# simplerr/rust-renderer

Measured on AMD Instinct MI355X. Metric: Mrays/s (path rays: primary + bounce + sun-shadow + light-shadow) at 1920x1080, 20 spp = 20 frames x 1 spp; camera and sun at rest, the one-off builds of the camera grid and the sun grid outside the timed region (value_with_grid_builds charges them to these frames, value_tree_walk uses neither grid), higher is better.
Workload: dtype f32

## Files before the change

### rust-renderer_amd/csrc/context.hip

```cpp
#include <hip/hip_runtime.h>
#include <rccl/rccl.h>
#include <dlfcn.h>

#include <algorithm>
#include <atomic>
#include <chrono>
#include <cstdlib>
#include <cmath>
#include <cstdio>
#include <cstring>
#include <string>
#include <thread>
#include <vector>

#include "bvh.h"
#include "context_internal.h"
#include "context_state.h"
#include "device_scan.h"
#include "device_types.h"
#include "utopian_hip.h"

using namespace uh;

namespace {
std::string g_create_error;
}

int fail(uh_ctx* c, int code, const std::string& msg) {
   if (c)
      c->err = msg;
   else
      g_create_error = msg;
   return code;
}

namespace {

void begin_timed(uh_ctx* c, int kind, hipStream_t stream = nullptr) {
   if (!stream) stream = c->stream;
   if (!c->time_kernels) return;
   EventPair ep;
   if (!c->free_events.empty()) {
      ep = c->free_events.back();
      c->free_events.pop_back();
   } else {
      (void)hipEventCreate(&ep.start);
      (void)hipEventCreate(&ep.stop);
   }
   ep.kind = kind;
   (void)hipEventRecord(ep.start, stream);
   c->pending.push_back(ep);
}
void end_timed(uh_ctx* c, hipStream_t stream = nullptr) {
   if (!c->time_kernels) return;
   (void)hipEventRecord(c->pending.back().stop, stream ? stream : c->stream);
}
void drain_timed(uh_ctx* c) {
   for (EventPair& ep : c->pending) {
      float ms = 0.0f;
      if (hipEventSynchronize(ep.stop) == hipSuccess && hipEventElapsedTime(&ms, ep.start, ep.stop) == hipSuccess) {
         c->ms_by_kind[ep.kind] += ms;
         if (ep.kind == 0) c->trace_closest_launches++;
         if (ep.kind == 4) c->trace_light_launches++;
      }
      c->free_events.push_back(ep);
   }
   c->pending.clear();
}

}

LaunchCfg cfg(uh_ctx* c) {
// ... 132 lines not shown
   c->d_meshes.release();
   c->d_obj_corners.release();
   c->d_world_corners.release();
   c->d_node_box.release();
   c->d_refit_meshes.release();
   c->d_src.release();
   c->d_tex.release();
   c->d_lut.release();
   c->d_sun_cells.release();
   c->d_sun_entries.release();
   c->d_sun_recs.release();
   c->d_sun_coarse.release();
   c->d_cam_cells.release();
   c->d_cam_entries.release();
   c->accumulation.release();
   c->gbuffer.release();
   c->output.release();
   for (auto& r : c->reservoirs) r.release();
   c->dstats.release();
   for (HostMesh& m : c->meshes) {
      if (m.d_verts) (void)hipFree(m.d_verts);
      if (m.d_indices) (void)hipFree(m.d_indices);
   }
   for (hipEvent_t ev : c->mupd.ev)
      if (ev) (void)hipEventDestroy(ev);
   c->mupd.table.release();
   c->mupd.flag.release();
   for (hipEvent_t ev : {c->iso.begin, c->iso.end})
      if (ev) (void)hipEventDestroy(ev);
   c->iso.counts.release();
   c->iso.chunks.release();
   c->iso.box.release();
   c->iso.total.release();
   destroy_graphs(c);
   for (auto& s : c->slots) s.destroy();
   for (hipEvent_t ev : c->ev_band)
      if (ev) (void)hipEventDestroy(ev);
   if (c->restir_stream) {
      for (hipEvent_t ev : {c->ev_restir, c->rs_start, c->rs_stop})
         if (ev) (void)hipEventDestroy(ev);
      (void)hipStreamDestroy(c->restir_stream);
      c->restir_stream = nullptr;
   }
   c->owned_pixels.release();
   c->tile_send.release();
   c->tile_recv.release();
   if (c->ev_compose) (void)hipEventDestroy(c->ev_compose);
   delete c;
}

int uh_add_texture_rgba8(uh_ctx* c, const uint8_t* pixels, uint32_t w, uint32_t h, uint32_t* out_index) {
   if (!c) return UH_ERR_INVALID_ARGUMENT;
   if (!pixels || !w || !h) return fail(c, UH_ERR_INVALID_ARGUMENT, "uh_add_texture_rgba8: null or empty texture");
   HIP_TRY(c, hipSetDevice(c->device));
   uchar4* dev = nullptr;
   HIP_TRY(c, hipMalloc((void**)&dev, (size_t)w * h * 4));
   const uint32_t tiles_x = (w % 8 == 0 && h % 8 == 0) ? w / 8 : 0;
   std::vector<uint8_t> tiled;
   const uint8_t* src = pixels;
   if (tiles_x) {
      tiled.resize((size_t)w * h * 4);
      for (uint32_t y = 0; y < h; y++)
         for (uint32_t x = 0; x < w; x++) {
            size_t at = ((size_t)((y >> 3) * tiles_x + (x >> 3)) << 6) + ((y & 7) << 3) + (x & 7);
            std::memcpy(&tiled[at * 4], &pixels[((size_t)y * w + x) * 4], 4);
         }
      src = tiled.data();
   }
   hipError_t e = hipMemcpy(dev, src, (size_t)w * h * 4, hipMemcpyHostToDevice);
   if (e != hipSuccess) {
      (void)hipFree(dev);
      return fail(c, UH_ERR_HIP, std::string("texture upload: ") + hipGetErrorString(e));
   }
   c->textures.push_back(uh_ctx::HostTex{w, h, dev, tiles_x});
   c->built = false;
   if (out_index) *out_index = (uint32_t)c->textures.size() - 1;
   return UH_OK;
}

int uh_add_light(uh_ctx* c, const UhGpuLight* light, uint32_t* out_index) {
   if (!c) return UH_ERR_INVALID_ARGUMENT;
   if (!light) return fail(c, UH_ERR_INVALID_ARGUMENT, "uh_add_light: null light");
   if (c->lights.size() >= UH_MAX_GPU_LIGHTS) return fail(c, UH_ERR_CAPACITY, "uh_add_light: more than 1024 lights (MAX_NUM_GPU_LIGHTS)");
   c->lights.push_back(*light);
   c->built = false;
   c->topology_valid = false;
   if (out_index) *out_index = (uint32_t)c->lights.size() - 1;
   return UH_OK;
}

int uh_get_num_lights(uh_ctx* c, uint32_t* out) {
   if (!c || !out) return UH_ERR_INVALID_ARGUMENT;
   *out = (uint32_t)c->lights.size();
   return UH_OK;
}

extern "C++" FrameParams make_params(uh_ctx* c, const UhViewUniformData& v) {
   FrameParams fp;
   std::memset(&fp, 0, sizeof(fp));
   std::memcpy(fp.inv_view, v.inverse_view, sizeof(fp.inv_view));
   std::memcpy(fp.inv_proj, v.inverse_projection, sizeof(fp.inv_proj));
   std::memcpy(fp.prev_pv, v.prev_frame_projection_view, sizeof(fp.prev_pv));
   float d = (v.sun_dir[0] * v.sun_dir[0] + v.sun_dir[1] * v.sun_dir[1]) + v.sun_dir[2] * v.sun_dir[2];
   float inv = 1.0f / std::sqrt(d);
   for (int a = 0; a < 3; a++) fp.sun_dir[a] = v.sun_dir[a] * inv;
   fp.W = c->W;
   fp.H = c->H;
   fp.frame_number = (uint32_t)(int32_t)((float)v.total_samples + v.time * 10000.0f);
   fp.batch_frames = 1;
   fp.frame_numbers[0] = fp.frame_number;
   fp.total_samples_of[0] = v.total_samples;
   fp.samples_per_frame = v.samples_per_frame;
   fp.total_samples = v.total_samples;
   fp.num_bounces = v.num_bounces;
   fp.accumulation_limit = v.accumulation_limit;
   fp.sky_enabled = v.sky_enabled;
   fp.sun_shadow_enabled = v.sun_shadow_enabled;
   fp.lights_enabled = v.lights_enabled;
   fp.use_ris = v.use_ris_light_sampling;
   fp.full_frame_restir = c->full_frame_restir ? 1u : 0u;
   fp.furnace = c->furnace ? 1u : 0u;
   fp.num_lights_used = v.num_lights < v.max_num_lights_used ? v.num_lights : v.max_num_lights_used;
   fp.temporal_enabled = v.temporal_reuse_enabled;
   fp.spatial_enabled = v.spatial_reuse_enabled;
   fp.tp_rank = c->tp_rank;
   fp.tp_world = c->tp_world;
   fp.tp_tile = c->tp_tile;
// ... 856 lines not shown
   else if (n == "sun_grid_build") {
      c->sun_device_build = value != 0;
      c->sun_attempted = false;
   } else if (n == "sun_grid_density") {
      if (!range(1, 4096)) return bad("(entries per triangle) must be 1..4096");
      c->sun_limits.entries_per_triangle = (double)value;
      c->sun_attempted = false;
   } else if (n == "sun_grid_max_walk") {
      if (!range(1, 4096)) return bad("(longest list a ray tests itself) must be 1..4096");
      c->sun_limits.max_walk = (uint32_t)value;
      c->sun_attempted = false;
   } else if (n == "sun_grid_max_mb") {
      if (!range(1, 65536)) return bad("must be 1..65536");
      c->sun_limits.max_entries = ((uint64_t)value << 20) / sizeof(SunGridEntry);
      c->sun_attempted = false;
   } else if (n == "sun_grid_force") {
      const SunGridLimits defaults;
      c->sun_limits.max_mean_list = value ? 1e30 : defaults.max_mean_list;
      c->sun_limits.max_fallback_area = value ? 2.0 : defaults.max_fallback_area;
      c->sun_attempted = false;
   } else if (n == "sun_grid_inline_max_mb") {
      if (!range(-1, 1 << 20)) return bad("must be -1 (auto: 4 x the packet array), 0 (off) .. 1048576");
      c->sun_inline_max_mb = value;
      c->sun_attempted = false;
   } else if (n == "sun_verdicts")
      c->sun_verdicts = value != 0;
   else if (n == "sun_grid_coarse") {
      if (!range(0, 6)) return bad("(log2 of the block edge in cells) must be 0..6");
      c->sun_coarse_shift = (uint32_t)value;
      c->sun_attempted = false;
   }
   else if (n == "camera_grid")
      c->cam_grid_enabled = value != 0;
   else if (n == "camera_grid_max_walk") {
      if (!range(1, 4096)) return bad("must be 1..4096");
      c->cam_limits.max_walk = (uint32_t)value;
      c->cam_attempted = false;
   } else if (n == "camera_grid_walk_whole") {
      if (!range(0, 65536)) return bad("must be 0..65536");
      c->cam_walk_whole = (uint32_t)value;
      c->cam_attempted = false;
   } else if (n == "camera_grid_max_mean_list_x10") {
      if (!range(1, 100000)) return bad("must be 1..100000");
      c->cam_limits.max_mean_list = value / 10.0;
      c->cam_attempted = false;
   } else if (n == "primary_implicit")
      c->primary_implicit = value != 0;
   else if (n == "full_frame_restir")
      c->full_frame_restir = value != 0;
   else if (n == "iso_reference_triangulation")
      c->iso_reference = value != 0;
   else if (n == "furnace")
      c->furnace = value != 0;
   else if (n == "shadow_map_size") {
      if (!range(16, 8192)) return bad("must be 16..8192");
      if ((uint32_t)value != c->shadow_map_size) {
         if (int st = sync_all(c)) return st;
         c->hy.shadow_maps([](auto& b, size_t) { b.release(); });
         c->hy.s_bins.geom = 0;
         c->hy.smap_size = 0;
      }
      c->shadow_map_size = (uint32_t)value;
   }
   else if (n == "overlap")
      c->overlap_miss = c->overlap_shadow = value != 0;
   else if (n == "batch_frames") {
      if (!range(0, (int)kMaxBatchFrames)) return bad("must be 0 (auto) .. 32");
      c->batch_frames = (uint32_t)value;
   } else if (n == "frames_in_flight") {
      if (!range(1, (int)kMaxSlots)) return bad("must be 1..8");
      (void)sync_all(c);
      c->frames_in_flight = (uint32_t)value;
      c->next_slot = 0;
   } else if (n == "fused_bounces") {
      if (!range(-1, 8)) return bad("must be 0 (off), 1 (on when no frame is in flight), -1 (always on) or 2..8 (as 1, and blocks per CU of its grid)");
      c->fused_bounces = value != 0;
      c->fused_always = value == -1;
      if (value >= 2) c->fused_blocks_per_cu = (uint32_t)value;
   } else if (n == "trace_blocks_per_cu") {
      if (!range(1, 8)) return bad("must be 1..8");
      c->closest_blocks_per_cu = c->shadow_blocks_per_cu = (uint32_t)value;
   } else
      return fail(c, UH_ERR_INVALID_ARGUMENT, "unknown option: " + n);
   return UH_OK;
}

int uh_set_tile_partition(uh_ctx* c, uint32_t rank, uint32_t world, uint32_t tile_size) {
   if (!c) return UH_ERR_INVALID_ARGUMENT;
   if (world == 0 || rank >= world || tile_size == 0) return fail(c, UH_ERR_INVALID_ARGUMENT, "uh_set_tile_partition: need rank < world, tile_size > 0");
   HIP_TRY(c, hipSetDevice(c->device));
   if (int st = sync_all(c)) return st;
   c->tp_rank = rank;
   c->tp_world = world;
   c->tp_tile = tile_size;
   c->n_owned = c->W * c->H;
   c->owned_pixels.release();
   if (world > 1) {
      const uint32_t tiles_x = (c->W + tile_size - 1) / tile_size;
      std::vector<uint32_t> own;
      own.reserve((size_t)c->W * c->H / world + 1);
      for (uint32_t y = 0; y < c->H; y++)
         for (uint32_t x = 0; x < c->W; x++)
            if (((y / tile_size) * tiles_x + x / tile_size) % world == rank) own.push_back(y * c->W + x);
      c->n_owned = (uint32_t)own.size();
      HIP_TRY(c, c->owned_pixels.alloc(own.size() ? own.size() : 1));
      if (!own.empty()) HIP_TRY(c, hipMemcpy(c->owned_pixels.p, own.data(), own.size() * 4, hipMemcpyHostToDevice));
// ... 381 lines not shown
```

### rust-renderer_amd/csrc/context_state.h

```cpp
#pragma once
#include <hip/hip_runtime.h>

#include <string>
#include <utility>
#include <vector>

#include "bvh.h"
#include "context_internal.h"
#include "device_types.h"
#include "utopian_hip.h"

using namespace uh;

struct HostMesh {
   std::vector<UhVertex> vertices;
   std::vector<uint32_t> indices;
   UhGpuMaterial material;
   float o2w[12];
   float w2o[9];
   bool iso = false, iso_reference = true;
   uint32_t iso_res = 0;
   float iso_lo = 0.0f, iso_hi = 0.0f;
   bool dev = false, host_valid = true;
   UhVertex* d_verts = nullptr;
// ... 153 lines not shown
      radf.release();
      pixcol.release();
      for (auto& q : queues) q.release();
      sun_lit.release();
      control.release();
      for (hipEvent_t* ev : {&ev_traced, &ev_missed, &ev_shaded, &ev_shadowed, &ev_side_done, &ev_acc, &frame_start, &frame_stop}) {
         if (*ev) (void)hipEventDestroy(*ev);
         *ev = nullptr;
      }
      if (side) (void)hipStreamDestroy(side);
      if (stream) (void)hipStreamDestroy(stream);
      stream = side = nullptr;
      ready = false;
   }
};

constexpr uint32_t kRestirBatch = 16;
constexpr int kSpatialRing = 2 * (int)kRestirBatch + 1;

struct uh_ctx {
   int device = 0;
   Slot slots[kMaxSlots];
   uint32_t frames_in_flight = 4;
   uint32_t batch_frames = 0;
   uint32_t next_slot = 0;
   uint32_t shard_cap = 0;
   hipEvent_t last_acc = nullptr;
   hipStream_t restir_stream = nullptr;
   hipEvent_t ev_restir = nullptr, rs_start = nullptr, rs_stop = nullptr;
   bool restir_recorded = false;
   int spatial_cur = 0;
   hipEvent_t spatial_reader[kSpatialRing] = {};
   uint32_t rp_rank = 0, rp_world = 1, rp_band_rows = 0;
   size_t res_stride = 0;
   UhRestirExchangeFn rp_exchange = nullptr;
   void* rp_user = nullptr;
   hipEvent_t ev_band[kSpatialRing] = {};
   void* rccl = nullptr;
   hipEvent_t t_start = nullptr, t_stop = nullptr;
   Slot* last_slot = nullptr;
   hipStream_t& stream = slots[0].stream;
   PathState& ps = slots[0].ps;
   DevBuf<Control>& control = slots[0].control;
   bool overlap_miss = true, overlap_shadow = true;
   uint32_t W = 0, H = 0;
   uint32_t num_cus = 256;
   uint32_t closest_blocks_per_cu = 5, shadow_blocks_per_cu = 5;
   uint32_t cam_walk_whole = 512;
   bool fused_bounces = true;
   bool fused_always = false;
   static constexpr uint32_t kFusedMaxPaths = 4u << 20;
   uint32_t fused_blocks_per_cu = 4;
   static constexpr uint32_t kSingleFrameBlocksPerCu = 4;
   std::string err;

   std::vector<HostMesh> meshes;
   std::vector<UhGpuLight> lights;
   struct HostTex {
      uint32_t w, h;
      uchar4* dev;
      uint32_t tiles_x;
   };
   std::vector<HostTex> textures;
   bool built = false;

   DevBuf<float4> d_nodes, d_tris, d_shade, d_lights;
   DevBuf<MeshShade> d_meshes;
   DevBuf<float> d_obj_corners, d_world_corners, d_node_box;
   DevBuf<RefitMesh> d_refit_meshes;
   std::vector<uint32_t> packet_keys;
   std::vector<uint32_t> level_start;
   bool topology_valid = false;
   bool device_build = false, src_valid = false;
   uint32_t device_build_kind = 1;
   uint32_t ploc_sah_top = 1024;
   static constexpr uint32_t kPlocRadius = 8;
   BuildSources d_src;
   std::vector<uint32_t> src_tris;
   std::vector<uint64_t> src_serial;
   struct IsoUpdate {
      DevBuf<uint32_t> counts, chunks, box;
      DevBuf<unsigned long long> total;
      hipEvent_t begin = nullptr, end = nullptr;
      UhIsosurfaceUpdateStats st{};
   } iso;
   std::vector<uint64_t> packet_serial;
   struct MeshUpdate {
      DevBuf<DeformMesh> table;
      DevBuf<uint32_t> flag;
      hipEvent_t ev[3] = {nullptr, nullptr, nullptr};
      UhMeshUpdateStats st{};
   } mupd;
   float refit_ms = 0.0f;
   DevBuf<TexInfo> d_tex;
   DevBuf<float> d_lut;
   SceneDev scene{};

   DevBuf<float4> accumulation, gbuffer;
   DevBuf<uchar4> output;
   DevBuf<UhReservoir> reservoirs[3], spatial_ring;
   DevBuf<float4> gb_ray_o, gb_ray_d, gb_hit;
   DevBuf<DeviceStats> dstats;
   Images im{};

   bool count_visits = false, time_kernels = false, full_frame_restir = false;
   bool iso_reference = true;
   uint32_t shadow_map_size = 4096;
   bool furnace = false;
   uint64_t frames = 0;
   float build_ms = 0.0f, last_frame_ms = 0.0f;
   float ms_by_kind[5] = {0, 0, 0, 0, 0};
   uint32_t trace_closest_launches = 0, trace_light_launches = 0;
   bool frame_timed = false;
   std::vector<EventPair> pending, free_events;
// ... 159 lines not shown
```

### rust-renderer_amd/csrc/device_math.h

```cpp
#pragma once
#include <hip/hip_runtime.h>

#include "device_types.h"

namespace uh {

struct V3 {
   float x, y, z;
};
__device__ __forceinline__ V3 v3(float x, float y, float z) { return V3{x, y, z}; }
__device__ __forceinline__ V3 operator+(V3 a, V3 b) { return v3(a.x + b.x, a.y + b.y, a.z + b.z); }
__device__ __forceinline__ V3 operator-(V3 a, V3 b) { return v3(a.x - b.x, a.y - b.y, a.z - b.z); }
__device__ __forceinline__ V3 operator*(V3 a, V3 b) { return v3(a.x * b.x, a.y * b.y, a.z * b.z); }
__device__ __forceinline__ V3 operator*(V3 a, float s) { return v3(a.x * s, a.y * s, a.z * s); }
__device__ __forceinline__ V3 operator*(float s, V3 a) { return v3(s * a.x, s * a.y, s * a.z); }
__device__ __forceinline__ V3 vneg(V3 a) { return v3(-a.x, -a.y, -a.z); }
__device__ __forceinline__ float dot3(V3 a, V3 b) { return (a.x * b.x + a.y * b.y) + a.z * b.z; }
__device__ __forceinline__ float length3(V3 a) { return sqrtf(dot3(a, a)); }
__device__ __forceinline__ V3 normalize3(V3 a) {
   float inv = 1.0f / sqrtf(dot3(a, a));
   return a * inv;
}
__device__ __forceinline__ V3 xyz(float4 v) { return v3(v.x, v.y, v.z); }

__device__ __forceinline__ float4 mat4_mul(const float* m, float x, float y, float z, float w) {
   float4 r;
   r.x = ((m[0] * x + m[4] * y) + m[8] * z) + m[12] * w;
   r.y = ((m[1] * x + m[5] * y) + m[9] * z) + m[13] * w;
   r.z = ((m[2] * x + m[6] * y) + m[10] * z) + m[14] * w;
   r.w = ((m[3] * x + m[7] * y) + m[11] * z) + m[15] * w;
   return r;
}

__device__ __forceinline__ uint32_t jenkins_hash(uint32_t x) {
   x += x << 10;
   x ^= x >> 6;
   x += x << 3;
   x ^= x >> 11;
   x += x << 15;
   return x;
}
__device__ __forceinline__ uint32_t init_rng(uint32_t px, uint32_t py, uint32_t resx, uint32_t frame) {
   float d = (float)px * 1.0f + (float)py * (float)resx;
   return jenkins_hash((uint32_t)d ^ jenkins_hash(frame));
}
__device__ __forceinline__ float random_float(uint32_t& s) {
   s = s * 747796405u + 1u;
   uint32_t word = ((s >> ((s >> 28) + 4u)) ^ s) * 277803737u;
   word = (word >> 22) ^ word;
   return (float)word * 2.3283064365386963e-10f;
}
__device__ __forceinline__ V3 random_point_in_unit_sphere(uint32_t& s) {
   for (;;) {
      float a = random_float(s), b = random_float(s), c = random_float(s);
      V3 p = v3(2.0f * a - 1.0f, 2.0f * b - 1.0f, 2.0f * c - 1.0f);
      if (dot3(p, p) < 1.0f) return p;
// ... 92 lines not shown
   float phaseR = 3.0f * (1.0f + costh * costh) / (16.0f * PI);
   float g = fminf(0.85f, 0.9381f);
   float k = 1.55f * g - 0.55f * g * g * g;
   float kcosth = k * costh;
   float phaseM = (1.0f - k * k) / ((4.0f * PI) * (1.0f - kcosth) * (1.0f - kcosth));
   V3 od = v3(0, 0, 0), rayleigh = v3(0, 0, 0), mie = v3(0, 0, 0);
   float prev = 0.0f;
   const float kLog2[16] = {0.0f,          -4.0f,         -3.0f,          -2.4150374993f, -2.0f,          -1.6780719051f, -1.4150374993f, -1.1926450779f,
                            -1.0f,         -0.8300749986f, -0.6780719051f, -0.5405683814f, -0.4150374993f, -0.2995602819f, -0.1926450779f, -0.0931094044f};
   for (int i = 0; i < 16; i++) {
      float ray_time = i == 0 ? 0.0f : __builtin_amdgcn_exp2f(exponent * kLog2[i]) * ray_length;
      float step = ray_time - prev;
      V3 p = start + dir * ray_time;
      V3 dens = atmosphere_density(atmosphere_height(p));
      od = od + dens * step;
      V3 both_t = absorb(od + integrate_optical_depth(p, light_dir));
      rayleigh = rayleigh + both_t * phaseR * dens.x * step;
      mie = mie + both_t * phaseM * dens.y * step;
      prev = ray_time;
   }
   return (rayleigh * C_RAYLEIGH() + mie * C_MIE()) * v3(1, 1, 1) * 20.0f;
}
}

typedef uint32_t u4_t __attribute__((ext_vector_type(4)));
typedef uint32_t u2_t __attribute__((ext_vector_type(2)));
__device__ __forceinline__ MeshShade lds_fetch(const MeshShade* lds) {
   const uint32_t at = (uint32_t)(uintptr_t)(__attribute__((address_space(3))) const MeshShade*)lds;
   u4_t q[5];
   asm volatile(
      "ds_read_b128 %0, %5\n\tds_read_b128 %1, %5 offset:16\n\tds_read_b128 %2, %5 offset:32\n\tds_read_b128 %3, %5 offset:48\n\t"
      "ds_read_b128 %4, %5 offset:64\n\ts_waitcnt lgkmcnt(0)"
      : "=&v"(q[0]), "=&v"(q[1]), "=&v"(q[2]), "=&v"(q[3]), "=&v"(q[4])
      : "v"(at)
      : "memory");
   MeshShade m;
   static_assert(sizeof(m) == sizeof(q), "five quads");
   __builtin_memcpy(&m, q, sizeof(m));
   return m;
}
__device__ __forceinline__ TexInfo lds_fetch(const TexInfo* lds) {
   const uint32_t at = (uint32_t)(uintptr_t)(__attribute__((address_space(3))) const TexInfo*)lds;
   struct {
      u4_t a;
      u2_t b;
   } q;
   asm volatile("ds_read_b128 %0, %2\n\tds_read_b64 %1, %2 offset:16\n\ts_waitcnt lgkmcnt(0)" : "=&v"(q.a), "=&v"(q.b) : "v"(at) : "memory");
   TexInfo t;
   static_assert(sizeof(TexInfo) == 24, "texture descriptor: a quad and a pair");
   __builtin_memcpy(&t, &q, sizeof(t));
   return t;
}

__device__ __forceinline__ int mirror_index(int i, int n) {
   int period = 2 * n;
   int m = i % period;
   if (m < 0) m += period;
   return m < n ? m : period - 1 - m;
}
template <typename Pre>
__device__ __forceinline__ V3 sample_texture_pre(const SceneDev& sc, const float* __restrict__ lut, uint32_t index, float u, float v, const TexInfo* lds_tex, uint32_t n_lds_tex,
                                                 Pre&& pre) {
   if (index >= sc.num_textures) {
      pre();
      return v3(1, 1, 1);
   }
   TexInfo t;
   if (lds_tex) {
      t = lds_fetch(lds_tex + (index < n_lds_tex ? index : 0u));
      if (index >= n_lds_tex) t = sc.textures[index];
   } else {
      t = sc.textures[index];
   }
   float x = u * (float)t.w - 0.5f, y = v * (float)t.h - 0.5f;
   if (!(fabsf(x) < 1e9f) || !(fabsf(y) < 1e9f)) {
      pre();
      return v3(0, 0, 0);
   }
   float fx = floorf(x), fy = floorf(y);
   float ax = x - fx, ay = y - fy;
   int x0 = mirror_index((int)fx, (int)t.w), x1 = mirror_index((int)fx + 1, (int)t.w);
   int y0 = mirror_index((int)fy, (int)t.h), y1 = mirror_index((int)fy + 1, (int)t.h);
   const bool tiled = t.tiles_x != 0;
   auto address = [&](int xx, int yy) {
      const uint32_t in_tiles = ((uint32_t)((yy >> 3) * (int)t.tiles_x + (xx >> 3)) << 6) + (uint32_t)(((yy & 7) << 3) + (xx & 7));
      const uint32_t in_rows = (uint32_t)yy * t.w + (uint32_t)xx;
      return tiled ? in_tiles : in_rows;
   };
   const uchar4* q00 = t.texels + address(x0, y0);
   const uchar4* q10 = t.texels + address(x1, y0);
   const uchar4* q01 = t.texels + address(x0, y1);
   const uchar4* q11 = t.texels + address(x1, y1);
   uint32_t w00, w10, w01, w11;
   pre();
   asm volatile(
      "global_load_dword %0, %4, off\n\tglobal_load_dword %1, %5, off\n\tglobal_load_dword %2, %6, off\n\tglobal_load_dword %3, %7, off\n\t"
      "s_waitcnt vmcnt(0)"
      : "=&v"(w00), "=&v"(w10), "=&v"(w01), "=&v"(w11)
      : "v"(q00), "v"(q10), "v"(q01), "v"(q11)
      : "memory");
   auto texel = [](uint32_t w) { return make_uchar4((unsigned char)(w & 0xffu), (unsigned char)((w >> 8) & 0xffu), (unsigned char)((w >> 16) & 0xffu), (unsigned char)(w >> 24)); };
   const uchar4 p00 = texel(w00), p10 = texel(w10), p01 = texel(w01), p11 = texel(w11);
   const V3 t00 = v3(lut[p00.x], lut[p00.y], lut[p00.z]), t10 = v3(lut[p10.x], lut[p10.y], lut[p10.z]);
   const V3 t01 = v3(lut[p01.x], lut[p01.y], lut[p01.z]), t11 = v3(lut[p11.x], lut[p11.y], lut[p11.z]);
   V3 a = t00 * (1.0f - ax) + t10 * ax;
   V3 b = t01 * (1.0f - ax) + t11 * ax;
   return a * (1.0f - ay) + b * ay;
}
__device__ __forceinline__ V3 sample_texture(const SceneDev& sc, const float* __restrict__ lut, uint32_t index, float u, float v, const TexInfo* lds_tex = nullptr,
                                             uint32_t n_lds_tex = 0) {
   return sample_texture_pre(sc, lut, index, u, v, lds_tex, n_lds_tex, [] {});
}

template <typename LightPtr>
__device__ __forceinline__ float target_function(LightPtr lights, uint32_t num_lights, int light_index, V3 hit_position) {
   if (light_index < 0 || (uint32_t)light_index >= num_lights) return 0.0f;
   float4 lp = lights[2 * light_index], li = lights[2 * light_index + 1];
   float d = length3(xyz(lp) - hit_position);
   float d2 = d * d;
   return luminance(v3(li.x / d2, li.y / d2, li.z / d2));
}
__device__ __forceinline__ void sample_light_uniform(uint32_t num_used, uint32_t& rng, int& idx, float& w) {
   idx = (int)(random_float(rng) * (float)num_used);
   w = 1.0f / (float)num_used;
}
__device__ __forceinline__ void finalize_resampling(UhReservoir& r, float p_hat) {
   r.W_X = (p_hat == 0.0f) ? 0.0f : (1.0f / p_hat) * r.W_sum / (float)r.M;
}
__device__ __forceinline__ void update_reservoir(uint32_t& rng, UhReservoir& r, int Xi, float w_i, int M) {
   r.W_sum += w_i;
   r.M += M;
   if (random_float(rng) * r.W_sum < w_i) r.Y = Xi;
}

__device__ __forceinline__ void primary_ray(const FrameParams& fp, uint32_t px, uint32_t py, float jx, float jy, V3& org, V3& dir) {
   float cx = (float)px + jx, cy = (float)py + jy;
   float u = cx / (float)fp.W, v = cy / (float)fp.H;
   v = 1.0f - v;
   float dx = u * 2.0f - 1.0f, dy = v * 2.0f - 1.0f;
   float4 o4 = mat4_mul(fp.inv_view, 0.0f, 0.0f, 0.0f, 1.0f);
   float4 tg = mat4_mul(fp.inv_proj, dx, dy, 1.0f, 1.0f);
   V3 nt = normalize3(v3(tg.x, tg.y, tg.z));
   float4 d4 = mat4_mul(fp.inv_view, nt.x, nt.y, nt.z, 0.0f);
   org = v3(o4.x, o4.y, o4.z);
   dir = v3(d4.x, d4.y, d4.z);
}

__device__ __forceinline__ void primary_state(const FrameParams& fp, uint32_t id, float4& ro, float4& rd) {
   const uint32_t f = id / fp.n_owned, k = id - f * fp.n_owned;
   const uint32_t pix = fp.owned_pixels ? fp.owned_pixels[k] : k;
   const uint32_t px = pix % fp.W, py = pix / fp.W;
   uint32_t rng = init_rng(px, py, fp.W, fp.frame_numbers[f]);
   const uint32_t seed = rng;
// ... 54 lines not shown
```

### rust-renderer_amd/csrc/device_types.h

```cpp
#pragma once
#include <hip/hip_runtime.h>

#include <cstdint>
#include <vector>

#include "bvh.h"
#include "sun_grid.h"
#include "utopian_hip.h"

namespace uh {

constexpr uint32_t kMaxBounces = 64;
constexpr uint32_t kQueueKinds = 5;
enum { Q_RAY = 0, Q_LIGHT = 1, Q_SUN_TREE = 2, Q_MISS = 3, Q_CAM_TREE = 4 };
constexpr uint32_t kLaunchSlots = kMaxBounces * 4 + 8;

constexpr uint32_t kShards = 32;
constexpr uint32_t kShardBits = 5;
static_assert((1u << kShardBits) == kShards, "kShards is a power of two");
__host__ __device__ inline uint32_t shard_of_run(uint32_t run) { return (run * 0x9E3779B1u) >> (32 - kShardBits); }

constexpr uint32_t kBounceStride = ((kMaxBounces + 1 + 31) / 32) * 32;
constexpr uint32_t kSlotStride = ((kLaunchSlots + 31) / 32) * 32;
struct Control {
   uint32_t q_count[kShards * kQueueKinds * kBounceStride];
   uint32_t cursor[kShards * kSlotStride];
};
__host__ __device__ inline uint32_t qc_index(uint32_t bounce, uint32_t kind, uint32_t shard) { return (shard * kQueueKinds + kind) * kBounceStride + bounce; }
__host__ __device__ inline uint32_t cursor_index(uint32_t slot, uint32_t shard) { return shard * kSlotStride + slot; }

struct DeviceStats {
   unsigned long long rays[UH_RAY_KINDS];
   unsigned long long nodes_visited, tris_tested, shadow_nodes_visited, shadow_tris_tested;
   unsigned long long closest_hits, misses;
   unsigned long long sun_tree_rays;
   unsigned long long cam_tree_rays;
   unsigned long long cam_tris_tested;
   unsigned long long sun_covered_rays;
   unsigned long long light_nodes_visited, light_tris_tested;
};

struct alignas(16) MeshShade {
   float w2o[9];
   uint32_t diffuse_map;
   float base_color[3];
   float type;
   float property;
   uint32_t pad;
   float metallic, roughness;
   float pad2[2];
};
static_assert(sizeof(MeshShade) == 80, "mesh shading record");

struct TexInfo {
   const uchar4* texels;
   uint32_t w, h;
   uint32_t tiles_x;
   uint32_t pad;
};

struct SceneDev {
   const uint4* nodes;
   const float4* tris;
   const float4* shade;
   const MeshShade* meshes;
   const TexInfo* textures;
   const float4* lights;
   const float* unorm_lut;
   uint32_t num_nodes, num_tris, num_meshes, num_textures, num_lights;
};

constexpr uint32_t kMaxBatchFrames = 32;

struct FrameParams {
   uint32_t batch_frames;
   uint32_t frame_numbers[kMaxBatchFrames];
   uint32_t total_samples_of[kMaxBatchFrames];
   const UhReservoir* spatial_of[kMaxBatchFrames];
   float inv_view[16], inv_proj[16], prev_pv[16];
   float sun_dir[3];
   uint32_t W, H, frame_number;
   uint32_t samples_per_frame, total_samples, num_bounces, accumulation_limit;
   uint32_t sky_enabled, sun_shadow_enabled, lights_enabled, use_ris, full_frame_restir;
   uint32_t primary_implicit;
   uint32_t sun_verdicts;
   uint32_t furnace;
   uint32_t num_lights_used;
   uint32_t temporal_enabled, spatial_enabled;
   uint32_t tp_rank, tp_world, tp_tile, tiles_x;
   const uint32_t* owned_pixels;
   uint32_t n_owned;
};

constexpr uint32_t kRecQuads = 4;
enum { REC_ORIGIN = 0, REC_DIR = 1, REC_THR = 2, REC_RAD = 3 };
struct PathRecs {
   float4* base;
   size_t plane;
};
struct PathState {
   PathRecs set[2];
   float4* hit;
   float4* radf;
   float4* pixcol;
   uint32_t* queue[5];
   unsigned long long* sun_lit;
   uint32_t shard_cap;
};
__host__ __device__ inline float4* rec_quad(const PathRecs& rec, uint32_t pos, int quad) { return rec.base + rec.plane * (size_t)quad + pos; }

struct RawRays {
// ... 289 lines not shown
```

### rust-renderer_amd/csrc/scene_build.hip

```cpp
#include <hip/hip_runtime.h>

#include <chrono>
#include <cmath>
#include <cstring>
#include <functional>
#include <string>
#include <thread>
#include <vector>

#include "bvh.h"
#include "bvh_invariants.h"
#include "context_internal.h"
#include "context_state.h"
#include "device_scan.h"
#include "device_types.h"
#include "utopian_hip.h"

using namespace uh;

namespace {

bool is_identity3x4(const float* m) {
   static const float I[12] = {1, 0, 0, 0, 0, 1, 0, 0, 0, 0, 1, 0};
   return std::memcmp(m, I, sizeof(I)) == 0;
// ... 37 lines not shown
   if (c->meshes.size() >= UH_MAX_GPU_MESHES) return fail(c, UH_ERR_CAPACITY, "uh_add_mesh: more than 1024 meshes (MAX_NUM_GPU_MESHES)");
   if (num_indices / 3 > (1u << kPrimBits)) return fail(c, UH_ERR_CAPACITY, "uh_add_mesh: more than 4 Mi triangles in one mesh");
   for (uint32_t i = 0; i < num_indices; i++)
      if (indices[i] >= num_vertices) return fail(c, UH_ERR_INVALID_ARGUMENT, "uh_add_mesh: index out of range");
   for (uint32_t i = 0; i < num_vertices; i++)
      if (!std::isfinite(vertices[i].pos[0]) || !std::isfinite(vertices[i].pos[1]) || !std::isfinite(vertices[i].pos[2]))
         return fail(c, UH_ERR_INVALID_ARGUMENT, "uh_add_mesh: vertex position is not finite");
   for (int i = 0; i < 12; i++)
      if (!std::isfinite(world3x4[i])) return fail(c, UH_ERR_INVALID_ARGUMENT, "uh_add_mesh: transform is not finite");
   HostMesh m;
   m.vertices.assign(vertices, vertices + num_vertices);
   m.indices.assign(indices, indices + num_indices);
   m.material = *material;
   set_transform(m, world3x4);
   c->meshes.push_back(std::move(m));
   c->built = false;
   c->topology_valid = false;
   c->src_valid = false;
   if (out_mesh_index) *out_mesh_index = (uint32_t)c->meshes.size() - 1;
   return UH_OK;
}

int uh_set_instance_transform(uh_ctx* c, uint32_t mesh_index, const float world3x4[12]) {
   if (!c) return UH_ERR_INVALID_ARGUMENT;
   if (mesh_index >= c->meshes.size() || !world3x4) return fail(c, UH_ERR_INVALID_ARGUMENT, "uh_set_instance_transform: bad mesh index");
   for (int i = 0; i < 12; i++)
      if (!std::isfinite(world3x4[i])) return fail(c, UH_ERR_INVALID_ARGUMENT, "uh_set_instance_transform: transform is not finite");
   set_transform(c->meshes[mesh_index], world3x4);
   c->built = false;
   return UH_OK;
}

static int upload_scene_tables(uh_ctx* c) {
   std::vector<MeshShade> ms(c->meshes.size());
   for (size_t i = 0; i < c->meshes.size(); i++) {
      const HostMesh& m = c->meshes[i];
      std::memcpy(ms[i].w2o, m.w2o, sizeof(m.w2o));
      ms[i].diffuse_map = m.material.diffuse_map;
      for (int a = 0; a < 3; a++) ms[i].base_color[a] = m.material.base_color_factor[a];
      ms[i].type = m.material.raytrace_properties[0];
      ms[i].property = m.material.raytrace_properties[1];
      ms[i].pad = 0;
      ms[i].metallic = m.material.metallic_factor;
      ms[i].roughness = m.material.roughness_factor;
      ms[i].pad2[0] = ms[i].pad2[1] = 0.0f;
   }
   std::vector<float4> lights(2 * c->lights.size());
   for (size_t i = 0; i < c->lights.size(); i++) {
      const UhGpuLight& l = c->lights[i];
      lights[2 * i] = make_float4(l.position[0], l.position[1], l.position[2], 0.0f);
      lights[2 * i + 1] = make_float4(l.intensity[0], l.intensity[1], l.intensity[2], 0.0f);
   }
   std::vector<TexInfo> tex(c->textures.size());
   for (size_t i = 0; i < tex.size(); i++) tex[i] = TexInfo{c->textures[i].dev, c->textures[i].w, c->textures[i].h, c->textures[i].tiles_x, 0};

   HIP_TRY(c, c->d_meshes.alloc(ms.size()));
   HIP_TRY(c, c->d_lights.alloc(lights.size()));
   HIP_TRY(c, c->d_tex.alloc(tex.size()));
   if (!ms.empty()) HIP_TRY(c, hipMemcpy(c->d_meshes.p, ms.data(), ms.size() * sizeof(MeshShade), hipMemcpyHostToDevice));
   if (!lights.empty()) HIP_TRY(c, hipMemcpy(c->d_lights.p, lights.data(), lights.size() * sizeof(float4), hipMemcpyHostToDevice));
   if (!tex.empty()) HIP_TRY(c, hipMemcpy(c->d_tex.p, tex.data(), tex.size() * sizeof(TexInfo), hipMemcpyHostToDevice));
   c->scene.meshes = c->d_meshes.p;
   c->scene.textures = c->d_tex.p;
   c->scene.lights = c->d_lights.p;
   c->scene.unorm_lut = c->d_lut.p;
   c->scene.num_meshes = (uint32_t)ms.size();
   c->scene.num_textures = (uint32_t)tex.size();
   c->scene.num_lights = (uint32_t)c->lights.size();
   return UH_OK;
}

static int build_on_device(uh_ctx* c);

static int ensure_host_mirrors(uh_ctx* c) {
   for (HostMesh& m : c->meshes) {
      if (!m.dev || m.host_valid) continue;
      m.vertices.resize(3 * (size_t)m.dev_tris);
      m.indices.resize(m.vertices.size());
      if (m.dev_tris) {
         HIP_TRY(c, hipMemcpy(m.vertices.data(), m.d_verts, m.vertices.size() * sizeof(UhVertex), hipMemcpyDeviceToHost));
         c->iso.st.host_geometry_bytes += m.vertices.size() * sizeof(UhVertex);
      }
      for (size_t i = 0; i < m.indices.size(); i++) m.indices[i] = (uint32_t)i;
      m.host_valid = true;
   }
   for (HostMesh& m : c->meshes) {
      if (!m.upd || m.host_valid) continue;
      HIP_TRY(c, hipMemcpy(m.vertices.data(), m.d_verts, m.vertices.size() * sizeof(UhVertex), hipMemcpyDeviceToHost));
      c->mupd.st.host_geometry_bytes += m.vertices.size() * sizeof(UhVertex);
      m.host_valid = true;
   }
   return UH_OK;
}
static void count_host_upload(uh_ctx* c, size_t bytes_per_triangle) {
   for (const HostMesh& m : c->meshes) {
      if (m.dev) c->iso.st.host_geometry_bytes += bytes_per_triangle * m.dev_tris;
      if (m.upd && m.host_valid) c->mupd.st.host_geometry_bytes += bytes_per_triangle * m.tris();
   }
}

struct TriVerts { const UhVertex* v[3]; };
static TriVerts tri_verts(const HostMesh& m, uint32_t p) {
   const uint32_t* ix = &m.indices[3 * (size_t)p];
   return TriVerts{{&m.vertices[ix[0]], &m.vertices[ix[1]], &m.vertices[ix[2]]}};
}
static void write_obj_corners(const TriVerts& t, float* o) {
   for (int k = 0; k < 3; k++)
// ... 690 lines not shown
```

Measured before the change: 10020.

## Store textures in overlapping blocks so bilinear taps need two paired loads

Adds a texture layout made of overlapping 8x4 blocks that share one edge texel with their neighbours, so every 2x2 bilinear footprint lies inside a single block. The sampler then fetches it with two dwordx2 loads (one per row) instead of four scattered dword loads, and picks the four texels with selects. The layout is on by default through a new texture_blocks option. It costs extra texture memory for the duplicated edges, a host-side repack at upload, and a cap on texture size.

```diff
diff --git a/rust-renderer_amd/csrc/context.hip b/rust-renderer_amd/csrc/context.hip
--- a/rust-renderer_amd/csrc/context.hip
+++ b/rust-renderer_amd/csrc/context.hip
@@ -18,6 +18,7 @@
 #include "context_state.h"
 #include "device_scan.h"
 #include "device_types.h"
+#include "texture_layout.h"
 #include "utopian_hip.h"
 
 using namespace uh;
@@ -256,27 +257,36 @@
 int uh_add_texture_rgba8(uh_ctx* c, const uint8_t* pixels, uint32_t w, uint32_t h, uint32_t* out_index) {
    if (!c) return UH_ERR_INVALID_ARGUMENT;
    if (!pixels || !w || !h) return fail(c, UH_ERR_INVALID_ARGUMENT, "uh_add_texture_rgba8: null or empty texture");
-   HIP_TRY(c, hipSetDevice(c->device));
-   uchar4* dev = nullptr;
-   HIP_TRY(c, hipMalloc((void**)&dev, (size_t)w * h * 4));
-   const uint32_t tiles_x = (w % 8 == 0 && h % 8 == 0) ? w / 8 : 0;
-   std::vector<uint8_t> tiled;
+   size_t texels = (size_t)w * h;
+   uint32_t tiles_x = 0, blocks_x = 0;
+   std::vector<uint8_t> packed;
    const uint8_t* src = pixels;
-   if (tiles_x) {
-      tiled.resize((size_t)w * h * 4);
+   if (c->texture_blocks) {
+      if (TexLayout::texel_count(w, h, &texels) != UH_OK)
+         return fail(c, UH_ERR_CAPACITY, "uh_add_texture_rgba8: the blocked texture would hold more than 2^32 texels (option texture_blocks = 0 stores it as it is)");
+      blocks_x = (uint32_t)TexLayout::blocks_x(w);
+      packed.resize(texels * 4);
+      TexLayout::repack(pixels, w, h, packed.data());
+      src = packed.data();
+   } else if (w % 8 == 0 && h % 8 == 0) {
+      tiles_x = w / 8;
+      packed.resize(texels * 4);
       for (uint32_t y = 0; y < h; y++)
          for (uint32_t x = 0; x < w; x++) {
             size_t at = ((size_t)((y >> 3) * tiles_x + (x >> 3)) << 6) + ((y & 7) << 3) + (x & 7);
-            std::memcpy(&tiled[at * 4], &pixels[((size_t)y * w + x) * 4], 4);
+            std::memcpy(&packed[at * 4], &pixels[((size_t)y * w + x) * 4], 4);
          }
-      src = tiled.data();
-   }
-   hipError_t e = hipMemcpy(dev, src, (size_t)w * h * 4, hipMemcpyHostToDevice);
+      src = packed.data();
+   }
+   HIP_TRY(c, hipSetDevice(c->device));
+   uchar4* dev = nullptr;
+   HIP_TRY(c, hipMalloc((void**)&dev, texels * 4));
+   hipError_t e = hipMemcpy(dev, src, texels * 4, hipMemcpyHostToDevice);
    if (e != hipSuccess) {
       (void)hipFree(dev);
       return fail(c, UH_ERR_HIP, std::string("texture upload: ") + hipGetErrorString(e));
    }
-   c->textures.push_back(uh_ctx::HostTex{w, h, dev, tiles_x});
+   c->textures.push_back(uh_ctx::HostTex{w, h, dev, tiles_x, blocks_x});
    c->built = false;
    if (out_index) *out_index = (uint32_t)c->textures.size() - 1;
    return UH_OK;
@@ -1239,6 +1249,8 @@
       c->iso_reference = value != 0;
    else if (n == "furnace")
       c->furnace = value != 0;
+   else if (n == "texture_blocks")
+      c->texture_blocks = value != 0;
    else if (n == "shadow_map_size") {
       if (!range(16, 8192)) return bad("must be 16..8192");
       if ((uint32_t)value != c->shadow_map_size) {
diff --git a/rust-renderer_amd/csrc/context_state.h b/rust-renderer_amd/csrc/context_state.h
--- a/rust-renderer_amd/csrc/context_state.h
+++ b/rust-renderer_amd/csrc/context_state.h
@@ -229,6 +229,7 @@
    static constexpr uint32_t kFusedMaxPaths = 4u << 20;
    uint32_t fused_blocks_per_cu = 4;
    static constexpr uint32_t kSingleFrameBlocksPerCu = 4;
+   bool texture_blocks = true;
    std::string err;
 
    std::vector<HostMesh> meshes;
@@ -237,6 +238,7 @@
       uint32_t w, h;
       uchar4* dev;
       uint32_t tiles_x;
+      uint32_t blocks_x;
    };
    std::vector<HostTex> textures;
    bool built = false;
diff --git a/rust-renderer_amd/csrc/device_math.h b/rust-renderer_amd/csrc/device_math.h
--- a/rust-renderer_amd/csrc/device_math.h
+++ b/rust-renderer_amd/csrc/device_math.h
@@ -2,6 +2,7 @@
 #include <hip/hip_runtime.h>
 
 #include "device_types.h"
+#include "texture_layout.h"
 
 namespace uh {
 
@@ -200,12 +201,6 @@
    return t;
 }
 
-__device__ __forceinline__ int mirror_index(int i, int n) {
-   int period = 2 * n;
-   int m = i % period;
-   if (m < 0) m += period;
-   return m < n ? m : period - 1 - m;
-}
 template <typename Pre>
 __device__ __forceinline__ V3 sample_texture_pre(const SceneDev& sc, const float* __restrict__ lut, uint32_t index, float u, float v, const TexInfo* lds_tex, uint32_t n_lds_tex,
                                                  Pre&& pre) {
@@ -229,24 +224,39 @@
    float ax = x - fx, ay = y - fy;
    int x0 = mirror_index((int)fx, (int)t.w), x1 = mirror_index((int)fx + 1, (int)t.w);
    int y0 = mirror_index((int)fy, (int)t.h), y1 = mirror_index((int)fy + 1, (int)t.h);
+   const bool blocked = t.blocks_x != 0;
+   const int mx = x0 < x1 ? x0 : x1, my = y0 < y1 ? y0 : y1;
    const bool tiled = t.tiles_x != 0;
    auto address = [&](int xx, int yy) {
       const uint32_t in_tiles = ((uint32_t)((yy >> 3) * (int)t.tiles_x + (xx >> 3)) << 6) + (uint32_t)(((yy & 7) << 3) + (xx & 7));
       const uint32_t in_rows = (uint32_t)yy * t.w + (uint32_t)xx;
       return tiled ? in_tiles : in_rows;
    };
-   const uchar4* q00 = t.texels + address(x0, y0);
-   const uchar4* q10 = t.texels + address(x1, y0);
-   const uchar4* q01 = t.texels + address(x0, y1);
-   const uchar4* q11 = t.texels + address(x1, y1);
+   const uchar4* q00 = t.texels + (blocked ? TexLayout::footprint_offset(t.blocks_x, (uint32_t)mx, (uint32_t)my) : address(x0, y0));
    uint32_t w00, w10, w01, w11;
    pre();
-   asm volatile(
-      "global_load_dword %0, %4, off\n\tglobal_load_dword %1, %5, off\n\tglobal_load_dword %2, %6, off\n\tglobal_load_dword %3, %7, off\n\t"
-      "s_waitcnt vmcnt(0)"
-      : "=&v"(w00), "=&v"(w10), "=&v"(w01), "=&v"(w11)
-      : "v"(q00), "v"(q10), "v"(q01), "v"(q11)
-      : "memory");
+   if (blocked) {
+      u2_t r0, r1;
+      asm volatile("global_load_dwordx2 %0, %2, off\n\tglobal_load_dwordx2 %1, %2, off offset:%3\n\ts_waitcnt vmcnt(0)"
+                   : "=&v"(r0), "=&v"(r1)
+                   : "v"(q00), "n"(TexLayout::kW * 4)
+                   : "memory");
+      const u2_t ra = y0 != my ? r1 : r0, rb = y1 != my ? r1 : r0;
+      w00 = x0 != mx ? ra.y : ra.x;
+      w10 = x1 != mx ? ra.y : ra.x;
+      w01 = x0 != mx ? rb.y : rb.x;
+      w11 = x1 != mx ? rb.y : rb.x;
+   } else {
+      const uchar4* q10 = t.texels + address(x1, y0);
+      const uchar4* q01 = t.texels + address(x0, y1);
+      const uchar4* q11 = t.texels + address(x1, y1);
+      asm volatile(
+         "global_load_dword %0, %4, off\n\tglobal_load_dword %1, %5, off\n\tglobal_load_dword %2, %6, off\n\tglobal_load_dword %3, %7, off\n\t"
+         "s_waitcnt vmcnt(0)"
+         : "=&v"(w00), "=&v"(w10), "=&v"(w01), "=&v"(w11)
+         : "v"(q00), "v"(q10), "v"(q01), "v"(q11)
+         : "memory");
+   }
    auto texel = [](uint32_t w) { return make_uchar4((unsigned char)(w & 0xffu), (unsigned char)((w >> 8) & 0xffu), (unsigned char)((w >> 16) & 0xffu), (unsigned char)(w >> 24)); };
    const uchar4 p00 = texel(w00), p10 = texel(w10), p01 = texel(w01), p11 = texel(w11);
    const V3 t00 = v3(lut[p00.x], lut[p00.y], lut[p00.z]), t10 = v3(lut[p10.x], lut[p10.y], lut[p10.z]);
diff --git a/rust-renderer_amd/csrc/device_types.h b/rust-renderer_amd/csrc/device_types.h
--- a/rust-renderer_amd/csrc/device_types.h
+++ b/rust-renderer_amd/csrc/device_types.h
@@ -56,7 +56,7 @@
    const uchar4* texels;
    uint32_t w, h;
    uint32_t tiles_x;
-   uint32_t pad;
+   uint32_t blocks_x;
 };
 
 struct SceneDev {
diff --git a/rust-renderer_amd/csrc/scene_build.hip b/rust-renderer_amd/csrc/scene_build.hip
--- a/rust-renderer_amd/csrc/scene_build.hip
+++ b/rust-renderer_amd/csrc/scene_build.hip
@@ -113,7 +113,7 @@
       lights[2 * i + 1] = make_float4(l.intensity[0], l.intensity[1], l.intensity[2], 0.0f);
    }
    std::vector<TexInfo> tex(c->textures.size());
-   for (size_t i = 0; i < tex.size(); i++) tex[i] = TexInfo{c->textures[i].dev, c->textures[i].w, c->textures[i].h, c->textures[i].tiles_x, 0};
+   for (size_t i = 0; i < tex.size(); i++) tex[i] = TexInfo{c->textures[i].dev, c->textures[i].w, c->textures[i].h, c->textures[i].tiles_x, c->textures[i].blocks_x};
 
    HIP_TRY(c, c->d_meshes.alloc(ms.size()));
    HIP_TRY(c, c->d_lights.alloc(lights.size()));
diff --git a/rust-renderer_amd/csrc/texture_layout.h b/rust-renderer_amd/csrc/texture_layout.h
--- /dev/null
+++ b/rust-renderer_amd/csrc/texture_layout.h
@@ -0,0 +1,68 @@
+#pragma once
+#include <stddef.h>
+#include <stdint.h>
+#include <string.h>
+
+#include "utopian_hip.h"
+
+#if defined(__HIPCC__)
+#define UH_HD __host__ __device__
+#else
+#define UH_HD
+#endif
+
+#ifndef UH_TEX_BLOCK_W
+#define UH_TEX_BLOCK_W 8
+#define UH_TEX_BLOCK_H 4
+#endif
+constexpr uint32_t kTexBlockW = UH_TEX_BLOCK_W, kTexBlockH = UH_TEX_BLOCK_H;
+
+namespace uh {
+
+UH_HD inline int mirror_index(int i, int n) {
+   int period = 2 * n;
+   int m = i % period;
+   if (m < 0) m += period;
+   return m < n ? m : period - 1 - m;
+}
+
+template <uint32_t W, uint32_t H>
+struct TexBlocks {
+   static_assert(W >= 2 && H >= 2, "a block holds a 2 x 2 footprint");
+   static constexpr uint32_t kW = W, kH = H, kTexels = W * H;
+
+   static UH_HD size_t blocks_x(size_t w) { return (w - 1) / (W - 1) + 1; }
+   static UH_HD size_t blocks_y(size_t h) { return (h - 1) / (H - 1) + 1; }
+   static int texel_count(uint32_t w, uint32_t h, size_t* out) {
+      if (!w || !h) return UH_ERR_INVALID_ARGUMENT;
+      const size_t blocks = blocks_x(w) * blocks_y(h);
+      if (blocks > (((size_t)1 << 32) / kTexels)) return UH_ERR_CAPACITY;
+      *out = blocks * kTexels;
+      return UH_OK;
+   }
+   static UH_HD uint32_t texel_offset(uint32_t blocks_per_row, uint32_t bx, uint32_t by, uint32_t col, uint32_t row) {
+      return (by * blocks_per_row + bx) * kTexels + row * W + col;
+   }
+   static UH_HD uint32_t footprint_offset(uint32_t blocks_per_row, uint32_t mx, uint32_t my) {
+      const uint32_t bx = mx / (W - 1), by = my / (H - 1);
+      return texel_offset(blocks_per_row, bx, by, mx - bx * (W - 1), my - by * (H - 1));
+   }
+   static void repack(const uint8_t* rgba, uint32_t w, uint32_t h, uint8_t* out) {
+      const size_t nbx = blocks_x(w), nby = blocks_y(h);
+      for (size_t by = 0; by < nby; by++)
+         for (size_t bx = 0; bx < nbx; bx++) {
+            uint8_t* block = out + (by * nbx + bx) * kTexels * 4;
+            for (size_t j = 0; j < H; j++) {
+               const size_t y = by * (H - 1) + j < h ? by * (H - 1) + j : (size_t)h - 1;
+               for (size_t i = 0; i < W; i++) {
+                  const size_t x = bx * (W - 1) + i < w ? bx * (W - 1) + i : (size_t)w - 1;
+                  memcpy(block + (j * W + i) * 4, rgba + (y * w + x) * 4, 4);
+               }
+            }
+         }
+   }
+};
+
+using TexLayout = TexBlocks<kTexBlockW, kTexBlockH>;
+
+}
```

New measurement: 10250, median of 6. 2.4% higher.
